# fanzhongyi/diffusion

Hardware: AMD Instinct MI355X
Metric: U-Net training images/sec @256 (SD-2-base U-Net, precomputed latents 4x32x32) (higher is better)
Workload: dtype bf16; 1 GPU; SD-2-base U-Net train step, latents 4x32x32, text 77x1024, batch 256/GPU (global 256), microbatch 256, AdamW, dp1; global_batch=256, microbatch=256, parallelism=dp1, params=865910724

## Files before the change

### diffusion_amd/_lib.py

```python
from __future__ import annotations

import ctypes as C
import os

_HERE = os.path.dirname(os.path.abspath(__file__))
LIB_PATH = os.path.join(_HERE, os.environ.get('DA_LIB_ALT') or 'libdiffusion_amd.so')

_vp, _l, _i, _f, _fp, _ll = C.c_void_p, C.c_long, C.c_int, C.c_float, C.c_void_p, C.c_void_p



class DaWgradItem(C.Structure):
    _fields_ = [('dY', C.c_void_p), ('lddy', C.c_long), ('X', C.c_void_p), ('ldx', C.c_long), ('dW', C.c_void_p),
                ('dbias', C.c_void_p), ('N', C.c_int), ('Cin', C.c_int)]


SIGNATURES = {
    'da_gemm_nt': [_vp, _l, _vp, _vp, _l, _fp, _vp, _l, _vp, _l, _i, _i, _i, _i, _i, _i, _i, _i, _i, _i, _i, _f, _fp, _l,
                   _vp],
    'da_set_option': [C.c_char_p, _i],
    'da_gemm_nt_variant_for': [_i, _i, _i, _i, _l],
    'da_gemm_nt_geglu': [_vp, _l, _vp, _vp, _l, _vp, _l, _fp, _i, _i, _i, _vp],
    'da_gemm_nt_geglu_bwd': [_vp, _l, _vp, _vp, _l, _vp, _l, _i, _i, _i, _vp],
    'da_gemm_tn_wgrad': [_vp, _l, _vp, _l, _fp, _fp, _fp, _i, _i, _i, _i, _i, _i, _i, _i, _i, _fp, _l, _vp],
    'da_gemm_tn_variant_for': [_i, _i, _i, _i, _i, _i, _i, _i, _i],
    'da_gemm_tn_wgrad_group': [C.POINTER(DaWgradItem), _i, _i, _fp, _l, _vp],
    'da_gemm_tn_group_plan': [C.POINTER(DaWgradItem), _i, _i, _l, C.POINTER(_i), _i, C.POINTER(_i)],
    'da_attn_fwd': [_vp, _l, _vp, _l, _vp, _l, _vp, _l, _fp, _i, _i, _i, _i, _f, _vp],
    'da_attn_fwd_causal': [_vp, _l, _vp, _l, _vp, _l, _vp, _l, _fp, _i, _i, _i, _f, _vp],
    'da_attn_fwd_wide': [_vp, _l, _vp, _l, _vp, _l, _vp, _l, _fp, _i, _i, _i, _i, _i, _f, _vp],
    'da_attn_bwd': [_vp, _l, _vp, _l, _vp, _l, _vp, _l, _vp, _l, _fp, _fp, _vp, _l, _vp, _l, _vp, _l, _i, _i, _i, _i,
                    _f, _vp],
    'da_norm_scratch_floats': [_i, _i, _i],
    'da_groupnorm_fwd': [_vp, _l, _vp, _l, _fp, _fp, _fp, _fp, _fp, _i, _i, _i, _i, _f, _i, _vp],
    'da_groupnorm_bwd': [_vp, _l, _vp, _l, _vp, _l, _vp, _l, _fp, _fp, _fp, _fp, _fp, _fp, _fp, _i, _i, _i, _i, _i,
                         _vp],
# ... 85 lines not shown
```

### diffusion_amd/csrc/gemm_nt.hip

```cpp
#include <string.h>

#include "common.hpp"
#include "diffusion_amd.h"

namespace {

struct GemmNTParams {
  const bf16* A;
  const bf16* W;
  void* C;
  const float* bias;
  const bf16* rowbias;
  const bf16* R;
  long lda, ldc, ldrb, ldr;
  int M, N, K, Cin;
  int Hin, Win, Hout, Wout;
  int ksize, mode;
  int out_fp32;
  float alpha;
  int tiles_m, tiles_n;
};

constexpr int BM = 128, BN = 128, BK = 64;
constexpr int STAGE_BYTES = (BM + BN) * BK * 2;
// ... 193 lines not shown
      }
    }
  }
}

}

int da_gemm_nt_v2_dispatch(int variant, int splits, float* ws, const void* A, long lda, const void* W, void* C, long ldc, const float* bias,
                           const void* rowbias, long ldrb, const void* R, long ldr, int M, int N, int K, int Cin,
                           int Hin, int Win, int Hout, int Wout, int ksize, int mode, int out_fp32, float alpha,
                           hipStream_t stream);

int da_gemm_nt_v3_try(const void* A, long lda, const void* W, void* C, long ldc, const float* bias, const void* R, long ldr,
                      int M, int N, int K, hipStream_t stream);
extern int g_nt_stream, g_nt_stream_lw;
int da_gemm_nt_ws_try(const void* A, long lda, const void* W, const float* bias, const void* R, long ldr, void* C, long ldc,
                      int M, int N, int K, hipStream_t stream);
extern int g_nt_ws;

extern int g_tn_variant;
extern int g_nt_korder;
extern int g_nt_persist;
extern int g_reserve_cus;
extern int g_nt_persist_conv;
extern int g_nt_de;
extern int g_grad_overwrite;
extern int g_attn_fused_bwd;
extern int g_tn_ring, g_tn_ungroup;
extern int g_gn_resident, g_gn_resident_form, g_gn_resident_min_slab;
int da_usable_cus(int cus);
// ... 52 lines not shown
        best_v = f.variant;
        best_s = s;
      }
    }
  }
  *splits = best_s;
  if (best_v == 12 && (g_nt_mfma32 == 1 || (g_nt_mfma32 < 0 && K <= 320))) return 15;
  return best_v;
}

extern "C" int da_gemm_nt_variant_for(int M, int N, int K, int Cin, long ws_floats) {
  int s;
  return pick_nt_variant(M, N, K, Cin, ws_floats, &s);
}

extern "C" int da_set_option(const char* key, int value) {
  if (key && !strcmp(key, "gemm_nt_variant")) {
    g_nt_variant = value;
    return DA_OK;
  }
  if (key && !strcmp(key, "gemm_nt_splitk")) {
    g_nt_splitk = value;
    return DA_OK;
  }
  if (key && !strcmp(key, "gemm_nt_dispatch")) {
    g_nt_dispatch = value;
    return DA_OK;
  }
  if (key && !strcmp(key, "gemm_nt_persist")) {
    g_nt_persist = value;
// ... 28 lines not shown
    if (value != 0 && value != 1) return DA_ERR_SHAPE;
    g_tn_ungroup = value;
    return DA_OK;
  }
  if (key && !strcmp(key, "gemm_nt_stream_lw")) {
    if (value != 4 && value != 16) return DA_ERR_SHAPE;
    g_nt_stream_lw = value;
    return DA_OK;
  }
  if (key && !strcmp(key, "gemm_nt_stream")) {
    g_nt_stream = value;
    return DA_OK;
  }
  if (key && !strcmp(key, "gemm_nt_de")) {
    g_nt_de = value;
    return DA_OK;
  }
  if (key && !strcmp(key, "gemm_nt_persist_conv")) {
    g_nt_persist_conv = value;
    return DA_OK;
  }
  if (key && !strcmp(key, "gn_resident")) {
    if (value < 0) return DA_ERR_SHAPE;
    g_gn_resident = value;
    return DA_OK;
  }
  if (key && !strcmp(key, "gn_resident_min_slab")) {
    if (value < 0) return DA_ERR_SHAPE;
    g_gn_resident_min_slab = value;
    return DA_OK;
// ... 29 lines not shown
  if (Hout <= 0 || Wout <= 0 || (M % (Hout * Wout))) return DA_ERR_SHAPE;
  if (R && (ldr & 7)) return DA_ERR_SHAPE;
  if (rowbias && (ldrb & 7)) return DA_ERR_SHAPE;
  if (g_nt_ws && g_nt_variant == 0 && ksize == 1 && mode == 0 && !out_fp32 && alpha == 1.0f && !rowbias) {
    const int rc = da_gemm_nt_ws_try(A, lda, W, bias, R, ldr, C, ldc, M, N, K, stream);
    if (rc >= 0) return rc;
  }
  if (g_nt_stream && g_nt_variant == 0 && ksize == 1 && mode == 0 && !out_fp32 && alpha == 1.0f && !rowbias &&
      (g_nt_stream == 2 || (K <= 640 && (long)((M + 127) / 128) * ((N + 319) / 320) >= 512))) {
    const int rc = da_gemm_nt_v3_try(A, lda, W, C, ldc, bias, R, ldr, M, N, K, stream);
    if (rc >= 0) return rc;
  }
  {
    int splits = 1;
    const int variant = pick_nt_variant(M, N, K, Cin, splitk_ws ? splitk_ws_floats : 0, &splits);
    if (variant != 1)
      return da_gemm_nt_v2_dispatch(variant, splits, splitk_ws, A, lda, W, C, ldc, bias, rowbias, ldrb, R, ldr, M, N, K, Cin, Hin, Win,
                                    Hout, Wout, ksize, mode, out_fp32, alpha, stream);
  }
  GemmNTParams p;
  p.A = (const bf16*)A; p.W = (const bf16*)W; p.C = C; p.bias = bias;
  p.rowbias = (const bf16*)rowbias; p.R = (const bf16*)R;
  p.lda = lda; p.ldc = ldc; p.ldrb = ldrb; p.ldr = ldr;
  p.M = M; p.N = N; p.K = K; p.Cin = Cin;
  p.Hin = Hin; p.Win = Win; p.Hout = Hout; p.Wout = Wout;
  p.ksize = ksize; p.mode = mode; p.out_fp32 = out_fp32; p.alpha = alpha;
  p.tiles_m = (M + BM - 1) / BM;
  p.tiles_n = (N + BN - 1) / BN;
  static unsigned long long attr_done = 0;
  if (da_ensure_dyn_smem((const void*)gemm_nt_kernel, SMEM_BYTES, &attr_done) != DA_OK) return DA_ERR_LAUNCH;
  hipLaunchKernelGGL(gemm_nt_kernel, dim3(p.tiles_m * p.tiles_n), dim3(256), SMEM_BYTES, stream, p);
  DA_CHECK_LAUNCH();
  return DA_OK;
}
```

### diffusion_amd/csrc/gemm_nt_v2.hip

```cpp
#include "common.hpp"
#include "diffusion_amd.h"
#ifndef NT2_NT
#define NT2_NT 0
#endif
#if NT2_NT
#define NTST st8_nt
#else
#define NTST st8
#endif


#ifndef NT2_CT
#define NT2_CT 1
#endif

int g_nt_persist = -1;
int g_reserve_cus = 0;
int g_nt_persist_conv = 1;
int g_nt_de = 1;
int da_usable_cus(int cus) {
  int n = cus - g_reserve_cus;
  return n < 32 ? 32 : n;
}

namespace {

struct GemmNT2Params {
  const bf16* A;
  const bf16* W;
  void* C;
  const float* bias;
  const bf16* rowbias;
  const bf16* R;
  long lda, ldc, ldrb, ldr;
  int M, N, K, Cin;
  int Hin, Win, Hout, Wout;
  int ksize, mode;
  int out_fp32;
  float alpha;
  int tiles_m, tiles_n;
  int splits, ksteps_per_split;
  long slab_stride;
  bf16* G;
  long ldg;
  int inner;
  int total_blocks;
  FastDiv div_hw, div_w;
  FastDiv div_nblk, div_tn;
  int korder;
};

__device__ __attribute__((aligned(256))) unsigned char g_zero_page[256];

template <int BK>
DEVINL int swz_key(int row) { return BK == 64 ? ((row >> 1) & 7) : ((row >> 2) & 3); }
template <int BK>
DEVINL int swz2(int row, int chunk) { return row * (BK * 2) + ((chunk ^ swz_key<BK>(row)) << 4); }

DEVINL void lds_barrier() {
  asm volatile("s_waitcnt lgkmcnt(0)" ::: "memory");
  __builtin_amdgcn_s_barrier();
  asm volatile("" ::: "memory");
}

// ... 4 lines not shown
    if (threadIdx.x == 0 && g_stamp_buf) g_stamp_buf[(long)vblock * 16 + (i)] = __builtin_amdgcn_s_memtime(); \
  } while (0)
extern "C" int da_debug_set_stamps(void* buf) {
  return hipMemcpyToSymbol(HIP_SYMBOL(g_stamp_buf), &buf, sizeof(buf)) == hipSuccess ? 0 : -1;
}
#else
#define STAMP(i) do {} while (0)
#endif

DEVINL void glds16(const void* gsrc, char* lds_dst) {
  __builtin_amdgcn_global_load_lds((const __attribute__((address_space(1))) void*)gsrc,
                                   (__attribute__((address_space(3))) void*)lds_dst, 16, 0, 0);
}

template <int MT, int NT, int WM, int WN, int BK, bool UPS, int GEGLU, bool EARLY, int MF = 16, bool PERSIST = EARLY, bool DE = false,
          bool HASR = false>
DEVINL void nt2_tile(const GemmNT2Params& p, const int vblock0, char* smem) {
  constexpr int NW = WM * WN;
  constexpr bool CT = MF == 16 && GEGLU == 0 && ((NT2_CT && !EARLY) || DE);
  static_assert(!DE || (MF == 16 && GEGLU == 0 && ((NT % 2) == 0 || (MT % 2) == 0)), "direct epilogue: 16x16 tiles in pairs");
  constexpr int V2_BM = MF * MT * WM, V2_BK = BK;
  static_assert((NW == 16 || NW == 8 || NW == 4) && (BK == 64 || BK == 32), "wave grid");
  static_assert(MF == 16 || (MF == 32 && GEGLU == 0 && BK == 64), "MFMA shape");
  constexpr int BN = MF * NT * WN;
  constexpr int SR = MF == 16 ? 16 : 8;
  constexpr int RG = 512 / BK;
  constexpr int LR = BK / 8;
  constexpr int AJ = V2_BM / RG / NW;
  constexpr int BGROUPS = BN / RG;
  constexpr int BJ = (BGROUPS + NW - 1) / NW;
  constexpr int A_BYTES = V2_BM * V2_BK * 2;
  constexpr int B_BYTES = BN * V2_BK * 2;
// ... 10 lines not shown
  const int wm = wave / WN, wn = wave % WN;
  auto task_of = [&](int ln, int pss, int tasks) {
    const bool ragged_last = (tasks % (64 * WN)) != 0 && pss == (tasks + 64 * WN - 1) / (64 * WN) - 1;
    const int slot = ragged_last ? (wn + WN - (wm * WN / 4) % WN) % WN : wn;
    return slot * 64 + ln + 64 * WN * pss;
  };
  auto fresh_lane = [&]() {
    int ln = lane;
    asm volatile("" : "+v"(ln));
    return ln;
  };
  STAMP(0);

  const int nblk = p.tiles_m * p.tiles_n;
  int split, tn, m0, n0;
  auto locate = [&](int vb) {
    split = (PERSIST && !EARLY) ? (int)fdiv((unsigned)vb, p.div_nblk) : vb / nblk;
    int bid = vb - split * nblk;
    const int q = nblk >> 3, r = nblk & 7;
    const int xcd = bid & 7, idx = bid >> 3;
    bid = (xcd < r ? xcd * (q + 1) : r * (q + 1) + (xcd - r) * q) + idx;
    const int tm = (PERSIST && !EARLY) ? (int)fdiv((unsigned)bid, p.div_tn) : bid / p.tiles_n;
    tn = bid - tm * p.tiles_n;
    m0 = tm * V2_BM;
    n0 = tn * BN;
  };
  auto wrow = [&](int c) {
    if constexpr (GEGLU == 1) return c < BN / 2 ? tn * (BN / 2) + c : p.inner + tn * (BN / 2) + (c - BN / 2);
    else return n0 + c;
  };
  const int HWo = p.Hout * p.Wout;
// ... 25 lines not shown
#pragma unroll
  for (int j = 0; j < AJ; ++j) {
    const int row = (wave * AJ + j) * RG + lrow;
    const int m = m0 + row;
    const bool mval = m < p.M;
    if constexpr (EARLY) {
#ifdef NT2_EXP_AHOT
      aoff[j] = (unsigned)(row) * (unsigned)(p.lda * 2) + (lchunk ^ swz_key<BK>(row)) * 16;
#else
      aoff[j] = (unsigned)(mval ? m : 0) * (unsigned)(p.lda * 2) + (lchunk ^ swz_key<BK>(row)) * 16;
#endif
      continue;
    }
    const int mm = mval ? m : 0;
    int b, rem, oh;
    if constexpr (PERSIST) {
      b = (int)fdiv((unsigned)mm, p.div_hw);
      rem = mm - b * HWo;
      oh = (int)fdiv((unsigned)rem, p.div_w);
    } else {
      b = mm / HWo;
      rem = mm - b * HWo;
      oh = rem / p.Wout;
    }
    const int ow = rem - oh * p.Wout;
    unsigned mask = ((oh & 1) << 16) | ((ow & 1) << 17);
    for (int t = 0; t < ntaps; ++t) {
      const int r = (PCONV || p.ksize == 3) ? t / 3 : 0, s2 = (PCONV || p.ksize == 3) ? t - 3 * r : 0;
      const int th = oh * gmul + r - pad, tw = ow * gmul + s2 - pad;
      const bool ok = mval && (unsigned)th < (unsigned)hlim && (unsigned)tw < (unsigned)wlim && !((th | tw) & pmask);
      mask |= (ok ? 1u : 0u) << t;
    }
    const int bh = (oh * gmul - pad) >> gshift, bw = (ow * gmul - pad) >> gshift;
    if constexpr (PERSIST && !UPS) {
// ... 1 lines not shown
      if (j == 0) amask[0] = mask & 0x1ffu;
      else amask[0] |= (mask & 0x1ffu) << (9 * j);
      continue;
    }
    amask[j] = mask;
    abase[j] = p.A + ((long)(b * p.Hin * p.Win) + (long)bh * p.Win + bw) * p.lda + (lchunk ^ swz_key<BK>(row)) * 8;
  }
#pragma unroll
  for (int j = 0; j < BJ; ++j) {
    const int g = wave + NW * j;
    const int row = g * RG + lrow;
    const int n = min(wrow(row), p.N - 1);
    woff[j] = ((unsigned)n * (unsigned)p.K + (lchunk ^ swz_key<BK>(row)) * 8) * 2;
  }

  const int kstep_begin = split * p.ksteps_per_split;
  nk = min(p.ksteps_per_split, nk_total - kstep_begin);
  if (tap_inner) {
    const int ch = kstep_begin / ntaps;
    tap = kstep_begin - ch * ntaps;
    c0 = ch * V2_BK;
  } else {
    const int kb = kstep_begin * V2_BK;
    tap = kb / p.Cin;
    c0 = kb - tap * p.Cin;
  }
  };
  auto issue = [&](int stage, bool live) {
    char* Ab = smem + stage * STAGE;
    char* Bb = Ab + A_BYTES;
// ... 30 lines not shown
        const long soff = (long)(dr * p.Win + ds) * p.lda + c0;
        const void* src = (amask[j] & tapbit) ? (const void*)(abase[j] + soff) : (const void*)zero;
        glds16(src, Ab + (wave * AJ + j) * 1024);
      }
    }
    const char* wb = reinterpret_cast<const char*>(p.W + (live ? tap * p.Cin + c0 : 0));
#pragma unroll
    for (int j = 0; j < BJ; ++j) {
      const int g = wave + NW * j;
      if constexpr (PERSIST && !EARLY) {
        if (BGROUPS % NW == 0 || g < BGROUPS) glds16(wb + (size_t)j * (NW * RG) * p.K * 2 + woff[0], Bb + g * 1024);
      } else {
        if (BGROUPS % NW == 0 || g < BGROUPS) glds16(wb + woff[j], Bb + g * 1024);
      }
    }
    const int tap_n = tap + 1, c_n = c0 + V2_BK;
    const bool wrap_t = tap_n >= ntaps, wrap_c = c_n >= p.Cin;
    if (tap_inner) {
      tap = wrap_t ? 0 : tap_n;
      c0 = wrap_t ? c_n : c0;
    } else {
      c0 = wrap_c ? 0 : c_n;
      tap = wrap_c ? tap_n : tap;
    }
  };

  typedef float accv_t __attribute__((ext_vector_type(MF == 16 ? 4 : 16)));
  accv_t acc[MT][NT];

  auto compute_half = [&](int stage, int s) {
    const char* Ab = smem + stage * STAGE;
    const char* Bb = Ab + A_BYTES;
// ... 96 lines not shown

  auto epilogue = [&](const int m0e, const int n0e, const int tne, const int splite, const int bbuf) {
  if constexpr (DE) {
    typedef unsigned u32x2_t __attribute__((ext_vector_type(2)));
    constexpr int NPJ = NT / 2;
    constexpr bool ODD = (NT & 1) != 0;
    constexpr int IH = ODD ? ((MT / 2 + 1) / 2) * 2 : (MT + 1) / 2;
    const int ln = fresh_lane();
    char* const cb = reinterpret_cast<char*>(p.C);
    const char* const rb = reinterpret_cast<const char*>(p.R);
    const int lrow = wm * (16 * MT) + (ln & 15), lq = (ln >> 4) & 1, lcol = wn * (16 * NT) + 8 * (ln >> 5);
    auto row_of = [&](int i) { return m0e + lrow + i * 16; };
    auto col_of = [&](int pj) { return n0e + lcol + 32 * pj + 16 * lq; };
    auto row5_of = [&](int i) { return m0e + lrow + (i - 1 + lq) * 16; };
    const int col5 = n0e + lcol + 16 * (NT - 1);
    u32x4 rin[MT][NPJ > 0 ? NPJ : 1], rin5[MT];
    auto fetch = [&](const int i_lo, const int i_hi) {
#pragma unroll
      for (int i = 0; i < MT; ++i) {
        if (i < i_lo || i >= i_hi) continue;
        const unsigned mo = (unsigned)min(row_of(i), p.M - 1) * (unsigned)(p.ldr * 2);
#pragma unroll
        for (int pj = 0; pj < NPJ; ++pj)
          rin[i][pj] = *reinterpret_cast<const u32x4*>(rb + (mo + (unsigned)min(col_of(pj), p.N - 8) * 2u));
        if constexpr (ODD) {
          if (i & 1)
            rin5[i] = *reinterpret_cast<const u32x4*>(rb + ((unsigned)min(row5_of(i), p.M - 1) * (unsigned)(p.ldr * 2) +
                                                            (unsigned)min(col5, p.N - 8) * 2u));
        }
      }
    };
    auto finish = [&](accv_t a, accv_t b, const u32x4 r, const int ma, const int mb, const int na, const int nb) {
      if (p.rowbias) {
        const int ia = (PERSIST && !EARLY) ? (int)fdiv((unsigned)min(ma, p.M - 1), p.div_hw) : min(ma, p.M - 1) / HWo;
        const int ib = (PERSIST && !EARLY) ? (int)fdiv((unsigned)min(mb, p.M - 1), p.div_hw) : min(mb, p.M - 1) / HWo;
        const bf16x4 ra = *reinterpret_cast<const bf16x4*>(p.rowbias + (long)ia * p.ldrb + min(na, p.N - 4));
        const bf16x4 rb4 = *reinterpret_cast<const bf16x4*>(p.rowbias + (long)ib * p.ldrb + min(nb, p.N - 4));
#pragma unroll
        for (int e = 0; e < 4; ++e) {
          a[e] += bf2f(ra[e]);
          b[e] += bf2f(rb4[e]);
        }
      }
      if constexpr (HASR) {
        const u32x2_t s0 = __builtin_amdgcn_permlane16_swap(r[0], r[2], false, false);
        const u32x2_t s1 = __builtin_amdgcn_permlane16_swap(r[1], r[3], false, false);
        a[0] += __builtin_bit_cast(float, s0[0] << 16);
// ... 17 lines not shown
#pragma unroll
    for (int i = 0; i < MT; ++i) {
      if constexpr (HASR) {
        if (i == IH) fetch(IH, MT);
      }
      const int m = row_of(i);
      const int ma = m0e + wm * (16 * MT) + i * 16 + (ln & 15);
#pragma unroll
      for (int pj = 0; pj < NPJ; ++pj) {
        const int n = col_of(pj);
        const int na = n0e + wn * (16 * NT) + 32 * pj + aq;
        const u32x4 o = finish(acc[i][2 * pj], acc[i][2 * pj + 1], rin[i][pj], ma, ma, na, na + 16);
#ifdef NT2_EXP_NOSTORE
        asm volatile("" ::"v"(o));
#else
        if (m < p.M && n < p.N) *reinterpret_cast<u32x4*>(cb + ((unsigned)m * (unsigned)(p.ldc * 2) + (unsigned)n * 2u)) = o;
#endif
      }
      if constexpr (ODD) {
        if (i & 1) {
          const int m5 = row5_of(i);
          const int na = n0e + wn * (16 * NT) + 16 * (NT - 1) + aq;
          const u32x4 o = finish(acc[i - 1][NT - 1], acc[i][NT - 1], rin5[i], ma - 16, ma, na, na);
#ifdef NT2_EXP_NOSTORE
          asm volatile("" ::"v"(o));
#else
          if (m5 < p.M && col5 < p.N) *reinterpret_cast<u32x4*>(cb + ((unsigned)m5 * (unsigned)(p.ldc * 2) + (unsigned)col5 * 2u)) = o;
#endif
        }
      }
    }
    STAMP(4);
    return;
  }
  const float* bias_lds = reinterpret_cast<const float*>(smem + BIAS_OFF + bbuf * (BN * 4));
  float* const strips = reinterpret_cast<float*>(smem + STRIP_OFF);
  const int el = fresh_lane();
  if constexpr (GEGLU == 1) {
    static_assert(BN == 320 && !UPS, "GEGLU tile = 160 value + 160 gate columns");
    constexpr int GLD = BN + 4, GSTRIP = 16 * GLD, HC = BN / 2;
    constexpr int GTASKS = 16 * (HC / 8), GPASSES = (GTASKS + 64 * WN - 1) / (64 * WN);
    const int mrow0g = m0e + wm * (16 * MT);
// ... 227 lines not shown
        locate(vnext);
        load_bias(bbuf ^ 1);
        describe();
        issue(0, true);
      }
      STAMP(8);
      epilogue(m0e, n0e, tne, splite, bbuf);
      STAMP(12);
      if (!more) break;
      vblock = vnext;
    }
  }
}

template <int MT, int NT, int WM, int WN, int BK, bool UPS, int GEGLU = 0, bool EARLY = false, int MF = 16, bool PERSIST = EARLY, bool DE = false,
          bool HASR = false>
__global__ __launch_bounds__(64 * WM * WN, (WM * WN == 16 ? 4 : 2)) void gemm_nt2_kernel(GemmNT2Params p) {
  extern __shared__ __attribute__((aligned(16))) char smem[];
  nt2_tile<MT, NT, WM, WN, BK, UPS, GEGLU, EARLY, MF, PERSIST, DE, HASR>(p, blockIdx.x, smem);
}

__global__ void splitk_finalize_kernel(GemmNT2Params p, const float* ws) {
  const int nvec = p.N >> 3;
  const long total = (long)p.M * nvec;
  const int HWo = p.Hout * p.Wout;
  for (long i = (long)blockIdx.x * blockDim.x + threadIdx.x; i < total; i += (long)gridDim.x * blockDim.x) {
    const long m = i / nvec;
    const int n = (int)(i - m * nvec) * 8;
    float v[8] = {0.f, 0.f, 0.f, 0.f, 0.f, 0.f, 0.f, 0.f};
#pragma unroll 4
    for (int s = 0; s < p.splits; ++s) {
      const float* src = ws + s * p.slab_stride + m * p.N + n;
      const f32x4 a = *reinterpret_cast<const f32x4*>(src), b = *reinterpret_cast<const f32x4*>(src + 4);
#pragma unroll
// ... 89 lines not shown
        hipLaunchKernelGGL((gemm_nt2_kernel<MT, NT, WM, WN, BK, UPS, 0, EARLY, MF, PERSIST, true, true>), dim3(grid), dim3(NTHREADS), SMEM, stream, p);
      } else {
        if (da_ensure_dyn_smem((const void*)gemm_nt2_kernel<MT, NT, WM, WN, BK, UPS, 0, EARLY, MF, PERSIST, true, false>, SMEM, &attr_done_de[0]) != DA_OK)
          return DA_ERR_LAUNCH;
        hipLaunchKernelGGL((gemm_nt2_kernel<MT, NT, WM, WN, BK, UPS, 0, EARLY, MF, PERSIST, true, false>), dim3(grid), dim3(NTHREADS), SMEM, stream, p);
      }
      DA_CHECK_LAUNCH();
      return DA_OK;
    }
  }
  hipLaunchKernelGGL((gemm_nt2_kernel<MT, NT, WM, WN, BK, UPS, 0, EARLY, MF, PERSIST>), dim3(grid), dim3(NTHREADS), SMEM, stream, p);
  DA_CHECK_LAUNCH();
  return DA_OK;
}

template <int GM>
int launch_v2_geglu(GemmNT2Params p, hipStream_t stream) {
  constexpr int BN = 320, STAGE = 256 * 64 * 2 + BN * 64 * 2, STRIPS = 4 * 16 * (BN + 4) * 4;
  constexpr int SMEM = (STAGE + STRIPS > 2 * STAGE ? STAGE + STRIPS : 2 * STAGE) + 2 * BN * 4;
  static_assert(SMEM <= 160 * 1024, "LDS");
  p.tiles_m = (p.M + 255) / 256;
  p.tiles_n = GM == 1 ? (p.inner + BN / 2 - 1) / (BN / 2) : (p.inner + BN - 1) / BN;
  p.splits = 1;
  p.ksteps_per_split = p.K / 64;
  static unsigned long long attr_done = 0;
  if (da_ensure_dyn_smem((const void*)gemm_nt2_kernel<4, 5, 4, 4, 64, false, GM, true>, SMEM, &attr_done) != DA_OK) return DA_ERR_LAUNCH;
  p.total_blocks = p.tiles_m * p.tiles_n;
  p.div_nblk = make_fastdiv((unsigned)p.total_blocks);
  p.div_tn = make_fastdiv((unsigned)p.tiles_n);
  if (p.total_blocks >= (1 << 20) || p.M >= (1 << 24)) return DA_ERR_SHAPE;
// ... 30 lines not shown
  GemmNT2Params p;
  p.A = (const bf16*)A; p.W = (const bf16*)W; p.C = C; p.bias = bias;
  p.rowbias = (const bf16*)rowbias; p.R = (const bf16*)R;
  p.lda = lda; p.ldc = ldc; p.ldrb = ldrb; p.ldr = ldr;
  p.M = M; p.N = N; p.K = K; p.Cin = Cin;
  p.Hin = Hin; p.Win = Win; p.Hout = Hout; p.Wout = Wout;
  p.ksize = ksize; p.mode = mode; p.out_fp32 = out_fp32; p.alpha = alpha;
  p.tiles_m = p.tiles_n = 0;
  p.splits = 1; p.ksteps_per_split = 0; p.slab_stride = 0;
  p.G = nullptr; p.ldg = 0; p.inner = 0;
  p.korder = g_nt_korder;
  p.total_blocks = 0;
  p.div_hw = make_fastdiv((unsigned)(Hout * Wout));
  p.div_w = make_fastdiv((unsigned)Wout);
  p.div_nblk = p.div_tn = make_fastdiv(1u);
  if (variant == 10) return launch_v2<8, 5, 2, 4, 64>(p, splits, ws, stream);
  if (variant == 11) return launch_v2<4, 10, 2, 2, 32>(p, 1, ws, stream);
  if (variant == 12) return launch_v2<4, 5, 4, 4, 64>(p, splits, ws, stream);
  if (variant == 15) return launch_v2<1, 5, 8, 2, 64, 32>(p, splits, ws, stream);
  if (variant == 16) return launch_v2<2, 5, 4, 2, 64, 32>(p, splits, ws, stream);
  if (variant == 18) return launch_v2<3, 4, 8, 2, 64>(p, splits, ws, stream);
  if (variant == 14) return launch_v2<4, 4, 4, 4, 64>(p, splits, ws, stream);
  return variant == 5 ? launch_v2<4, 5, 4, 2, 64>(p, splits, ws, stream) : launch_v2<4, 4, 4, 2, 64>(p, splits, ws, stream);
}

int da_gemm_nt_geglu_ws_try(const void* A, long lda, const void* W, const float* bias, void* F, long ldf, void* G, long ldg,
                            int M, int inner, int K, hipStream_t stream);

extern "C" int da_gemm_nt_geglu(const void* A, long lda, const void* W, void* F, long ldf, void* G, long ldg,
                                const float* bias, int M, int inner, int K, hipStream_t stream) {
  DA_CLEAR_ERR();
  if (M <= 0 || inner <= 0 || K <= 0) return DA_ERR_SHAPE;
  if ((inner % 160) || (K % 64) || (lda & 7) || (ldf & 7) || (ldg & 7)) return DA_ERR_SHAPE;
  if ((long)M * lda * 2 >= (1L << 32) || (long)inner * K * 4 >= (1L << 32)) return DA_ERR_SHAPE;
  {
    const int rc = da_gemm_nt_geglu_ws_try(A, lda, W, bias, F, ldf, G, ldg, M, inner, K, stream);
    if (rc >= 0) return rc;
  }
  GemmNT2Params p;
  p.A = (const bf16*)A; p.W = (const bf16*)W; p.C = F; p.bias = bias;
  p.rowbias = nullptr; p.R = nullptr;
  p.lda = lda; p.ldc = ldf; p.ldrb = 0; p.ldr = 0;
  p.M = M; p.N = 2 * inner; p.K = K; p.Cin = K;
  p.Hin = 1; p.Win = 1; p.Hout = 1; p.Wout = 1;
  p.ksize = 1; p.mode = 0; p.out_fp32 = 0; p.alpha = 1.0f;
  p.tiles_m = p.tiles_n = 0;
  p.splits = 1; p.ksteps_per_split = 0; p.slab_stride = 0;
  p.G = (bf16*)G; p.ldg = ldg; p.inner = inner; p.korder = 0; p.total_blocks = 0;
  p.div_hw = p.div_w = p.div_nblk = p.div_tn = make_fastdiv(1u);
  return launch_v2_geglu<1>(p, stream);
}

extern "C" int da_gemm_nt_geglu_bwd(const void* dY, long lddy, const void* Wt, const void* F, long ldf, void* dF, long lddf,
                                    int M, int inner, int K, hipStream_t stream) {
  DA_CLEAR_ERR();
  if (M <= 0 || inner <= 0 || K <= 0) return DA_ERR_SHAPE;
  if ((inner % 320) || (K % 64) || (lddy & 7) || (ldf & 7) || (lddf & 7)) return DA_ERR_SHAPE;
  if ((long)M * lddy * 2 >= (1L << 32) || (long)inner * K * 2 >= (1L << 32)) return DA_ERR_SHAPE;
  GemmNT2Params p;
  p.A = (const bf16*)dY; p.W = (const bf16*)Wt; p.C = dF; p.bias = nullptr;
  p.rowbias = nullptr; p.R = nullptr;
  p.lda = lddy; p.ldc = lddf; p.ldrb = 0; p.ldr = 0;
  p.M = M; p.N = inner; p.K = K; p.Cin = K;
  p.Hin = 1; p.Win = 1; p.Hout = 1; p.Wout = 1;
  p.ksize = 1; p.mode = 0; p.out_fp32 = 0; p.alpha = 1.0f;
  p.tiles_m = p.tiles_n = 0;
  p.splits = 1; p.ksteps_per_split = 0; p.slab_stride = 0;
  p.G = (bf16*)const_cast<void*>(F); p.ldg = ldf; p.inner = inner; p.korder = 0; p.total_blocks = 0;
  p.div_hw = p.div_w = p.div_nblk = p.div_tn = make_fastdiv(1u);
  return launch_v2_geglu<2>(p, stream);
}
```

### diffusion_amd/models/unet.py

```python
from __future__ import annotations

import math
import os
from dataclasses import dataclass
from typing import Dict, List, Optional, Tuple

import torch
import torch.nn as nn

from .. import ops
from ..ops import BF16, F32, Geom


@dataclass
class UNetConfig:
    in_channels: int = 4
    out_channels: int = 4
    block_out_channels: Tuple[int, ...] = (320, 640, 1280, 1280)
    attention_head_dim: Tuple[int, ...] = (5, 10, 20, 20)
    cross_attention_dim: int = 1024
    layers_per_block: int = 2
    norm_num_groups: int = 32
    norm_eps: float = 1e-5
    sample_size: int = 64
# ... 838 lines not shown
                self._wgrad(dpred, a, m.gw, g3, dbias=self.V('conv_out.bias').g, scratch=self._scratch)
                da = self._bf(B * H * W, m.C)
                ops.gemm_nt(dpred, m.wt, da, g3)
                dh = self._gn_bwd(h, da, None, 'conv_norm_out', st, B, H * W, 1)
            elif kind == 'resnet':
                dh = self._resnet_bwd(sv, dh)
                lo = off(sv[0] + '.norm1.weight')
            elif kind == 'transformer':
                dh = self._transformer_bwd(sv, dh)
                lo = off(sv[0] + '.norm.weight')
            elif kind == 'up':
                key, x, B, rh, rw = sv
                lo = off(key + '.weight')
                m = self.M(key + '.weight')
                self._wgrad(dh, x, m.gw, Geom.up(B, rh, rw), dbias=self.V(key + '.bias').g, scratch=self._scratch)
                dup = self._bf(B * 4 * rh * rw, m.C)
                ops.gemm_nt(dh, m.wt, dup, Geom.conv(B, 2 * rh, 2 * rw))
                dx = self._bf(B * rh * rw, m.C)
                ops.upsample2x_bwd(dup, dx, B, rh, rw, m.C)
                dh = dx
            elif kind == 'cat':
                s, cb = sv
                dskip[s] = dh[:, cb:]
                dh = dh[:, :cb]
            elif kind == 'skip':
                (s,) = sv
                tot = self._bf(*dh.shape)
                ops.add(dh, dskip.pop(s), tot)
                dh = tot
            elif kind == 'down':
                key, x, B, rh, rw = sv
                lo = off(key + '.weight')
                m = self.M(key + '.weight')
                self._wgrad(dh, x, m.gw, Geom.down(B, rh, rw), dbias=self.V(key + '.bias').g, scratch=self._scratch)
# ... 63 lines not shown
```

### diffusion_amd/ops.py

```python
from __future__ import annotations

import ctypes
import os
from typing import Optional, Tuple

import torch

from . import _lib

BF16 = torch.bfloat16
F32 = torch.float32


def _stream() -> int:
    return torch.cuda.current_stream().cuda_stream


SPLITK_WS = None


PROFILE = None


class _Timed:
# ... 122 lines not shown
                14: 'gemm_nt2_kernel<4,4,4,4>', 15: 'gemm_nt2_kernel<1,5,8,2,mf32>', 16: 'gemm_nt2_kernel<2,5,4,2,mf32>',
                18: 'gemm_nt2_kernel<3,4,8,2>'}[v]
        ws = _opt('gemm_nt_ws', 1)
        ws_bn = 320 if (K == 320 and (ws & 1) and N <= 1280) else 128 if (K == 640 and (ws & 2) and N <= 1024) else 0
        if (ws_bn and _opt('gemm_nt_variant', 0) == 0 and N % ws_bn == 0 and M % 32 == 0 and (M // 32) * (N // ws_bn) >= 8 * 256
                and g.ksize == 1 and g.mode == 0 and not out_fp32 and alpha == 1.0 and rowbias is None):
            name = 'gemm_nt_ws_kernel'
    with _Timed(name, flops, (M, N, K, g.ksize, g.mode)):
        _lib.call('da_gemm_nt', a_ptr, lda, w_ptr, c_ptr, ldc, _vec(bias, N, 'bias'), rb_ptr, ldrb, r_ptr, ldr, M, N,
                  K, Cin, g.Hin, g.Win, g.Hout, g.Wout, g.ksize, g.mode, int(out_fp32), float(alpha),
                  SPLITK_WS.data_ptr() if SPLITK_WS is not None else 0,
                  SPLITK_WS.numel() if SPLITK_WS is not None else 0, _stream())
    return out


def geglu_fusable(inner: int, K: int) -> bool:
    return inner % 160 == 0 and K % 64 == 0


def gemm_nt_geglu(A, W, F, G, bias):
    a_ptr, lda = _mat(A, BF16, 'A')
    w_ptr, ldw = _mat(W, BF16, 'W')
    f_ptr, ldf = _mat(F, BF16, 'F')
    g_ptr, ldg = _mat(G, BF16, 'G')
    M, K = A.shape
    inner = G.shape[1]
    if tuple(W.shape) != (2 * inner, K) or ldw != K or tuple(F.shape) != (M, 2 * inner) or G.shape[0] != M:
        raise ValueError('gemm_nt_geglu: shape mismatch')
    if not geglu_fusable(inner, K):
        raise ValueError(f'gemm_nt_geglu needs inner % 160 == 0 and K % 64 == 0, got {inner}, {K}')
# ... 660 lines not shown
```

### include/diffusion_amd.h

```cpp
#ifndef DIFFUSION_AMD_H
#define DIFFUSION_AMD_H

#ifdef __cplusplus
extern "C" {
#endif

typedef struct ihipStream_t* da_stream_t;

int da_gemm_nt(const void* A, long lda, const void* W, void* C, long ldc, const float* bias, const void* rowbias,
               long ldrb, const void* R, long ldr, int M, int N, int K, int Cin, int Hin, int Win, int Hout, int Wout,
               int ksize, int mode, int out_fp32, float alpha, float* splitk_ws, long splitk_ws_floats,
               da_stream_t stream);

int da_gemm_nt_geglu(const void* A, long lda, const void* W, void* F, long ldf, void* G, long ldg, const float* bias,
                     int M, int inner, int K, da_stream_t stream);

int da_gemm_nt_geglu_bwd(const void* dY, long lddy, const void* Wt, const void* F, long ldf, void* dF, long lddf, int M,
                         int inner, int K, da_stream_t stream);

int da_set_option(const char* key, int value);
int da_gemm_nt_variant_for(int M, int N, int K, int Cin, long splitk_ws_floats);

int da_gemm_tn_wgrad(const void* dY, long lddy, const void* X, long ldx, float* dW, float* dbias, float* scratch, int M,
                     int N, int Cin, int Hin, int Win, int Hout, int Wout, int ksize, int mode, float* split_ws,
                     long split_ws_floats, da_stream_t stream);

int da_gemm_tn_variant_for(int M, int N, int Cin, int Hin, int Win, int Hout, int Wout, int ksize, int mode);

typedef struct DaWgradItem {
  const void* dY;
  long lddy;
  const void* X;
  long ldx;
  float* dW;
  float* dbias;
  int N;
// ... 145 lines not shown
```

Baseline: 1517 images/sec.

## Add parity-class upsample conv and fold upsample backward into dgrad GEMM

Measured after the change: 1523 images/sec, median of 6. No clear change (+0.4%).

```diff
diff --git a/diffusion_amd/_lib.py b/diffusion_amd/_lib.py
--- a/diffusion_amd/_lib.py
+++ b/diffusion_amd/_lib.py
@@ -20,6 +20,8 @@
                    _vp],
     'da_set_option': [C.c_char_p, _i],
     'da_gemm_nt_variant_for': [_i, _i, _i, _i, _l],
+    'da_gemm_nt_form_launches': [_i],
+    'da_gemm_nt_up_fold': [_vp, _l, _vp, _vp, _l, _fp, _i, _i, _i, _i, _i, _l, _vp],
     'da_gemm_nt_geglu': [_vp, _l, _vp, _vp, _l, _vp, _l, _fp, _i, _i, _i, _vp],
     'da_gemm_nt_geglu_bwd': [_vp, _l, _vp, _vp, _l, _vp, _l, _i, _i, _i, _vp],
     'da_gemm_tn_wgrad': [_vp, _l, _vp, _l, _fp, _fp, _fp, _i, _i, _i, _i, _i, _i, _i, _i, _i, _fp, _l, _vp],
diff --git a/diffusion_amd/csrc/gemm_nt.hip b/diffusion_amd/csrc/gemm_nt.hip
--- a/diffusion_amd/csrc/gemm_nt.hip
+++ b/diffusion_amd/csrc/gemm_nt.hip
@@ -231,6 +231,13 @@
 int da_gemm_nt_v3_try(const void* A, long lda, const void* W, void* C, long ldc, const float* bias, const void* R, long ldr,
                       int M, int N, int K, hipStream_t stream);
 extern int g_nt_stream, g_nt_stream_lw;
+int da_gemm_nt_s2c_try(const void* A, long lda, const void* W, void* C, long ldc, const float* bias, const void* rowbias, const void* R,
+                       int M, int N, int K, int Cin, int Hin, int Win, int Hout, int Wout, int ksize, int mode, int out_fp32, float alpha,
+                       hipStream_t stream);
+int da_gemm_nt_upf_try(const void* dY, long lddy, const void* Wt, void* dX, long lddx, const float* bias, int B, int H, int W, int N, int Cin,
+                       hipStream_t stream);
+extern int g_nt_s2_classes, g_nt_up_fold;
+extern long g_nt_s2_launches, g_nt_upf_launches;
 int da_gemm_nt_ws_try(const void* A, long lda, const void* W, const float* bias, const void* R, long ldr, void* C, long ldc,
                       int M, int N, int K, hipStream_t stream);
 extern int g_nt_ws;
@@ -313,6 +320,11 @@
   return pick_nt_variant(M, N, K, Cin, ws_floats, &s);
 }
 
+extern "C" int da_gemm_nt_form_launches(int form) {
+  if (form != 0 && form != 1) return -1;
+  return (int)((form ? g_nt_upf_launches : g_nt_s2_launches) & 0x7fffffff);
+}
+
 extern "C" int da_set_option(const char* key, int value) {
   if (key && !strcmp(key, "gemm_nt_variant")) {
     g_nt_variant = value;
@@ -371,6 +383,16 @@
   }
   if (key && !strcmp(key, "gemm_nt_de")) {
     g_nt_de = value;
+    return DA_OK;
+  }
+  if (key && !strcmp(key, "gemm_nt_s2_classes")) {
+    if (value != 0 && value != 1) return DA_ERR_SHAPE;
+    g_nt_s2_classes = value;
+    return DA_OK;
+  }
+  if (key && !strcmp(key, "gemm_nt_up_fold")) {
+    if (value != 0 && value != 1) return DA_ERR_SHAPE;
+    g_nt_up_fold = value;
     return DA_OK;
   }
   if (key && !strcmp(key, "gemm_nt_persist_conv")) {
@@ -430,6 +452,11 @@
   {
     int splits = 1;
     const int variant = pick_nt_variant(M, N, K, Cin, splitk_ws ? splitk_ws_floats : 0, &splits);
+    if (g_nt_s2_classes && g_nt_variant == 0 && mode == 2 && splits == 1 &&
+        (variant == 4 || variant == 5 || variant == 12 || variant == 14 || variant == 18)) {
+      const int rc = da_gemm_nt_s2c_try(A, lda, W, C, ldc, bias, rowbias, R, M, N, K, Cin, Hin, Win, Hout, Wout, ksize, mode, out_fp32, alpha, stream);
+      if (rc >= 0) return rc;
+    }
     if (variant != 1)
       return da_gemm_nt_v2_dispatch(variant, splits, splitk_ws, A, lda, W, C, ldc, bias, rowbias, ldrb, R, ldr, M, N, K, Cin, Hin, Win,
                                     Hout, Wout, ksize, mode, out_fp32, alpha, stream);
@@ -449,3 +476,15 @@
   DA_CHECK_LAUNCH();
   return DA_OK;
 }
+
+extern "C" int da_gemm_nt_up_fold(const void* dY, long lddy, const void* Wt, void* dX, long lddx, const float* bias, int B, int H, int W, int N,
+                                  int Cin, long splitk_ws_floats, hipStream_t stream) {
+  DA_CLEAR_ERR();
+  if (B <= 0 || H <= 0 || W <= 0 || N <= 0 || Cin <= 0 || (long)B * 4 * H * W >= (1L << 31)) return DA_ERR_SHAPE;
+  if ((N & 7) || (Cin & 7) || (lddy & 7) || (lddx & 7)) return DA_ERR_SHAPE;
+  if (!g_nt_up_fold || g_nt_variant != 0) return -1;
+  int splits = 1;
+  const int variant = pick_nt_variant(B * 4 * H * W, N, 9 * Cin, Cin, splitk_ws_floats, &splits);
+  if (splits != 1 || !(variant == 4 || variant == 5 || variant == 12 || variant == 14 || variant == 18)) return -1;
+  return da_gemm_nt_upf_try(dY, lddy, Wt, dX, lddx, bias, B, H, W, N, Cin, stream);
+}
diff --git a/diffusion_amd/csrc/gemm_nt_v2.hip b/diffusion_amd/csrc/gemm_nt_v2.hip
--- a/diffusion_amd/csrc/gemm_nt_v2.hip
+++ b/diffusion_amd/csrc/gemm_nt_v2.hip
@@ -18,6 +18,9 @@
 int g_reserve_cus = 0;
 int g_nt_persist_conv = 1;
 int g_nt_de = 1;
+int g_nt_s2_classes = 1;
+int g_nt_up_fold = 1;
+long g_nt_s2_launches = 0, g_nt_upf_launches = 0;
 int da_usable_cus(int cus) {
   int n = cus - g_reserve_cus;
   return n < 32 ? 32 : n;
@@ -48,6 +51,7 @@
   FastDiv div_hw, div_w;
   FastDiv div_nblk, div_tn;
   int korder;
+  int s2_tmc;
 };
 
 __device__ __attribute__((aligned(256))) unsigned char g_zero_page[256];
@@ -82,8 +86,10 @@
 }
 
 template <int MT, int NT, int WM, int WN, int BK, bool UPS, int GEGLU, bool EARLY, int MF = 16, bool PERSIST = EARLY, bool DE = false,
-          bool HASR = false>
+          bool HASR = false, bool S2C = false, bool UPF = false>
 DEVINL void nt2_tile(const GemmNT2Params& p, const int vblock0, char* smem) {
+  static_assert(!S2C || (DE && !HASR && !PERSIST && !EARLY && !UPS && GEGLU == 0 && BK == 64), "parity-class form");
+  static_assert(!UPF || (DE && !HASR && !S2C && !EARLY && !UPS && GEGLU == 0 && BK == 64), "block-sum form");
   constexpr int NW = WM * WN;
   constexpr bool CT = MF == 16 && GEGLU == 0 && ((NT2_CT && !EARLY) || DE);
   static_assert(!DE || (MF == 16 && GEGLU == 0 && ((NT % 2) == 0 || (MT % 2) == 0)), "direct epilogue: 16x16 tiles in pairs");
@@ -124,7 +130,22 @@
 
   const int nblk = p.tiles_m * p.tiles_n;
   int split, tn, m0, n0;
+  int cls = 0;
   auto locate = [&](int vb) {
+    if constexpr (S2C) {
+      const int nct = p.s2_tmc * p.tiles_n;
+      cls = vb / nct;
+      int bid = vb - cls * nct;
+      const int q = nct >> 3, r = nct & 7;
+      const int xcd = bid & 7, idx = bid >> 3;
+      bid = (xcd < r ? xcd * (q + 1) : r * (q + 1) + (xcd - r) * q) + idx;
+      const int tm = bid / p.tiles_n;
+      split = 0;
+      tn = bid - tm * p.tiles_n;
+      m0 = tm * V2_BM;
+      n0 = tn * BN;
+      return;
+    }
     split = (PERSIST && !EARLY) ? (int)fdiv((unsigned)vb, p.div_nblk) : vb / nblk;
     int bid = vb - split * nblk;
     const int q = nblk >> 3, r = nblk & 7;
@@ -180,10 +201,28 @@
     }
     const int mm = mval ? m : 0;
     int b, rem, oh;
-    if constexpr (PERSIST) {
+    if constexpr (UPF) {
+      const int ql = mm >> 2, hwl = HWo >> 2, wl = p.Wout >> 1;
+      int lh;
+      if constexpr (PERSIST) {
+        b = (int)fdiv((unsigned)ql, p.div_hw);
+        lh = (int)fdiv((unsigned)(ql - b * hwl), p.div_w);
+      } else {
+        b = ql / hwl;
+        lh = (ql - b * hwl) / wl;
+      }
+      oh = 2 * lh + ((mm >> 1) & 1);
+      rem = oh * p.Wout + 2 * (ql - b * hwl - lh * wl) + (mm & 1);
+    } else if constexpr (PERSIST) {
       b = (int)fdiv((unsigned)mm, p.div_hw);
       rem = mm - b * HWo;
       oh = (int)fdiv((unsigned)rem, p.div_w);
+    } else if constexpr (S2C) {
+      const int hwl = p.Hin * p.Win;
+      b = mm / hwl;
+      const int reml = mm - b * hwl, lh = reml / p.Win;
+      oh = 2 * lh + (~cls & 1);
+      rem = oh * p.Wout + 2 * (reml - lh * p.Win) + ((~cls >> 1) & 1);
     } else {
       b = mm / HWo;
       rem = mm - b * HWo;
@@ -215,6 +254,13 @@
     woff[j] = ((unsigned)n * (unsigned)p.K + (lchunk ^ swz_key<BK>(row)) * 8) * 2;
   }
 
+  if constexpr (S2C) {
+    const int py = ~cls & 1, px = (~cls >> 1) & 1;
+    nk = (1 + py) * (1 + px) * (p.Cin / V2_BK);
+    tap = (py ? 0 : 3) + (px ? 0 : 1);
+    c0 = 0;
+    return;
+  }
   const int kstep_begin = split * p.ksteps_per_split;
   nk = min(p.ksteps_per_split, nk_total - kstep_begin);
   if (tap_inner) {
@@ -275,8 +321,26 @@
         if (BGROUPS % NW == 0 || g < BGROUPS) glds16(wb + woff[j], Bb + g * 1024);
       }
     }
-    const int tap_n = tap + 1, c_n = c0 + V2_BK;
-    const bool wrap_t = tap_n >= ntaps, wrap_c = c_n >= p.Cin;
+    const int c_n = c0 + V2_BK;
+    const bool wrap_c = c_n >= p.Cin;
+    if constexpr (S2C) {
+      const int py = ~cls & 1, px = (~cls >> 1) & 1;
+      int tap_n = (py ? 0 : 3) + (px ? 0 : 1);
+      bool wrap_t = false;
+      if (px && s2 == 0) tap_n = tap + 2;
+      else if (py && r == 0) tap_n = 6 + (px ? 0 : 1);
+      else wrap_t = true;
+      if (tap_inner) {
+        tap = tap_n;
+        c0 = wrap_t ? c_n : c0;
+      } else {
+        c0 = wrap_c ? 0 : c_n;
+        tap = wrap_c ? tap_n : tap;
+      }
+      return;
+    }
+    const int tap_n = tap + 1;
+    const bool wrap_t = tap_n >= ntaps;
     if (tap_inner) {
       tap = wrap_t ? 0 : tap_n;
       c0 = wrap_t ? c_n : c0;
@@ -403,6 +467,16 @@
     auto col_of = [&](int pj) { return n0e + lcol + 32 * pj + 16 * lq; };
     auto row5_of = [&](int i) { return m0e + lrow + (i - 1 + lq) * 16; };
     const int col5 = n0e + lcol + 16 * (NT - 1);
+    auto crow = [&](int m) {
+      if constexpr (S2C) {
+        const int g = m / p.Win;
+        return (unsigned)((2 * g + (~cls & 1)) * p.Wout + 2 * (m - g * p.Win) + ((~cls >> 1) & 1));
+      } else if constexpr (UPF) {
+        return (unsigned)(m >> 2);
+      } else {
+        return (unsigned)m;
+      }
+    };
     u32x4 rin[MT][NPJ > 0 ? NPJ : 1], rin5[MT];
     auto fetch = [&](const int i_lo, const int i_hi) {
 #pragma unroll
@@ -419,7 +493,23 @@
         }
       }
     };
+    auto block_sum = [&](const float v) {
+      const int x = __builtin_bit_cast(int, bf2f(f2bf(v)));
+      float sum = 0.f;
+      sum += __builtin_bit_cast(float, __builtin_amdgcn_update_dpp(0, x, 0x00, 0xf, 0xf, false));
+      sum += __builtin_bit_cast(float, __builtin_amdgcn_update_dpp(0, x, 0x55, 0xf, 0xf, false));
+      sum += __builtin_bit_cast(float, __builtin_amdgcn_update_dpp(0, x, 0xaa, 0xf, 0xf, false));
+      sum += __builtin_bit_cast(float, __builtin_amdgcn_update_dpp(0, x, 0xff, 0xf, 0xf, false));
+      return sum;
+    };
     auto finish = [&](accv_t a, accv_t b, const u32x4 r, const int ma, const int mb, const int na, const int nb) {
+      if constexpr (UPF) {
+#pragma unroll
+        for (int e = 0; e < 4; ++e) {
+          a[e] = block_sum(a[e]);
+          b[e] = block_sum(b[e]);
+        }
+      }
       if (p.rowbias) {
         const int ia = (PERSIST && !EARLY) ? (int)fdiv((unsigned)min(ma, p.M - 1), p.div_hw) : min(ma, p.M - 1) / HWo;
         const int ib = (PERSIST && !EARLY) ? (int)fdiv((unsigned)min(mb, p.M - 1), p.div_hw) : min(mb, p.M - 1) / HWo;
@@ -467,7 +557,7 @@
 #ifdef NT2_EXP_NOSTORE
         asm volatile("" ::"v"(o));
 #else
-        if (m < p.M && n < p.N) *reinterpret_cast<u32x4*>(cb + ((unsigned)m * (unsigned)(p.ldc * 2) + (unsigned)n * 2u)) = o;
+        if (m < p.M && n < p.N && (!UPF || (ln & 3) == 0)) *reinterpret_cast<u32x4*>(cb + (crow(m) * (unsigned)(p.ldc * 2) + (unsigned)n * 2u)) = o;
 #endif
       }
       if constexpr (ODD) {
@@ -478,7 +568,7 @@
 #ifdef NT2_EXP_NOSTORE
           asm volatile("" ::"v"(o));
 #else
-          if (m5 < p.M && col5 < p.N) *reinterpret_cast<u32x4*>(cb + ((unsigned)m5 * (unsigned)(p.ldc * 2) + (unsigned)col5 * 2u)) = o;
+          if (m5 < p.M && col5 < p.N && (!UPF || (ln & 3) == 0)) *reinterpret_cast<u32x4*>(cb + (crow(m5) * (unsigned)(p.ldc * 2) + (unsigned)col5 * 2u)) = o;
 #endif
         }
       }
@@ -736,10 +826,10 @@
 }
 
 template <int MT, int NT, int WM, int WN, int BK, bool UPS, int GEGLU = 0, bool EARLY = false, int MF = 16, bool PERSIST = EARLY, bool DE = false,
-          bool HASR = false>
+          bool HASR = false, bool S2C = false, bool UPF = false>
 __global__ __launch_bounds__(64 * WM * WN, (WM * WN == 16 ? 4 : 2)) void gemm_nt2_kernel(GemmNT2Params p) {
   extern __shared__ __attribute__((aligned(16))) char smem[];
-  nt2_tile<MT, NT, WM, WN, BK, UPS, GEGLU, EARLY, MF, PERSIST, DE, HASR>(p, blockIdx.x, smem);
+  nt2_tile<MT, NT, WM, WN, BK, UPS, GEGLU, EARLY, MF, PERSIST, DE, HASR, S2C, UPF>(p, blockIdx.x, smem);
 }
 
 __global__ void splitk_finalize_kernel(GemmNT2Params p, const float* ws) {
@@ -859,6 +949,65 @@
   return DA_OK;
 }
 
+int launch_v2_s2c(GemmNT2Params p, hipStream_t stream) {
+  constexpr int BM = 256, BN = 320, STAGE = BM * 64 * 2 + BN * 64 * 2, SMEM = 2 * STAGE + BN * 4;
+  if (p.mode != 2 || p.ksize != 3 || p.R || p.rowbias || p.out_fp32 || p.alpha != 1.0f) return -1;
+  if (p.Hout != 2 * p.Hin || p.Wout != 2 * p.Win || (p.M % (p.Hout * p.Wout)) || (p.Cin % 64) || p.K != 9 * p.Cin) return -1;
+  if ((p.N % 8) || (p.ldc % 8) || ((uintptr_t)p.C & 15) || (long)p.M * p.ldc * 2 >= (1L << 32) || (long)p.N * p.K * 2 >= (1L << 32)) return -1;
+  p.M /= 4;
+  p.s2_tmc = (p.M + BM - 1) / BM;
+  p.tiles_m = 4 * p.s2_tmc;
+  p.tiles_n = (p.N + BN - 1) / BN;
+  p.splits = 1;
+  p.ksteps_per_split = p.K / 64;
+  p.slab_stride = 0;
+  p.total_blocks = p.tiles_m * p.tiles_n;
+  static unsigned long long attr_done = 0;
+  if (da_ensure_dyn_smem((const void*)gemm_nt2_kernel<4, 5, 4, 4, 64, false, 0, false, 16, false, true, false, true>, SMEM, &attr_done) != DA_OK)
+    return DA_ERR_LAUNCH;
+  hipLaunchKernelGGL((gemm_nt2_kernel<4, 5, 4, 4, 64, false, 0, false, 16, false, true, false, true>), dim3(p.total_blocks), dim3(1024), SMEM, stream, p);
+  DA_CHECK_LAUNCH();
+  ++g_nt_s2_launches;
+  return DA_OK;
+}
+
+template <bool PERS>
+int launch_v2_upf_form(GemmNT2Params p, hipStream_t stream) {
+  constexpr int BM = 256, BN = 320, STAGE = BM * 64 * 2 + BN * 64 * 2, STRIPS = 4 * 16 * (BN + 4) * 4;
+  constexpr int SMEM = PERS ? (STAGE + STRIPS > 2 * STAGE ? STAGE + STRIPS : 2 * STAGE) + 2 * BN * 4 : 2 * STAGE + BN * 4;
+  static_assert(SMEM <= 160 * 1024, "LDS");
+  p.tiles_m = (p.M + BM - 1) / BM;
+  p.tiles_n = (p.N + BN - 1) / BN;
+  p.splits = 1;
+  p.ksteps_per_split = p.K / 64;
+  p.slab_stride = 0;
+  p.total_blocks = p.tiles_m * p.tiles_n;
+  p.div_nblk = make_fastdiv((unsigned)p.total_blocks);
+  p.div_tn = make_fastdiv((unsigned)p.tiles_n);
+  p.div_hw = make_fastdiv((unsigned)(p.Hout * p.Wout / 4));
+  p.div_w = make_fastdiv((unsigned)(p.Wout / 2));
+  if (PERS && p.total_blocks >= (1 << 20)) return -1;
+  static unsigned long long attr_done = 0;
+  if (da_ensure_dyn_smem((const void*)gemm_nt2_kernel<4, 5, 4, 4, 64, false, 0, false, 16, PERS, true, false, false, true>, SMEM, &attr_done) != DA_OK)
+    return DA_ERR_LAUNCH;
+  const int grid = PERS ? persistent_grid(p.total_blocks) : p.total_blocks;
+  hipLaunchKernelGGL((gemm_nt2_kernel<4, 5, 4, 4, 64, false, 0, false, 16, PERS, true, false, false, true>), dim3(grid), dim3(1024), SMEM, stream, p);
+  DA_CHECK_LAUNCH();
+  ++g_nt_upf_launches;
+  return DA_OK;
+}
+
+int launch_v2_upf(const GemmNT2Params& p, hipStream_t stream) {
+  if (p.mode != 0 || p.ksize != 3 || p.R || p.rowbias || p.out_fp32 || p.alpha != 1.0f) return -1;
+  if (p.Hin != p.Hout || p.Win != p.Wout || (p.Hout & 1) || (p.Wout & 1) || (p.M % (p.Hout * p.Wout)) || (p.Cin % 64) || p.K != 9 * p.Cin) return -1;
+  if ((p.N % 8) || (p.ldc % 8) || ((uintptr_t)p.C & 15) || (long)(p.M / 4) * p.ldc * 2 >= (1L << 32) || (long)p.N * p.K * 2 >= (1L << 32)) return -1;
+  const long tiles = (long)((p.M + 255) / 256) * ((p.N + 319) / 320);
+  if (g_nt_persist_conv && g_nt_persist != 0 && tiles > da_usable_cus(256) && p.N % 320 == 0 && p.M < (1 << 24) &&
+      (long)p.M * p.Hout * p.Wout < (1L << 40) && (long)(p.M / (p.Hout * p.Wout)) * p.Hin * p.Win * p.lda * 2 < (1L << 32))
+    return launch_v2_upf_form<true>(p, stream);
+  return launch_v2_upf_form<false>(p, stream);
+}
+
 template <int GM>
 int launch_v2_geglu(GemmNT2Params p, hipStream_t stream) {
   constexpr int BN = 320, STAGE = 256 * 64 * 2 + BN * 64 * 2, STRIPS = 4 * 16 * (BN + 4) * 4;
@@ -919,6 +1068,9 @@
   p.div_hw = make_fastdiv((unsigned)(Hout * Wout));
   p.div_w = make_fastdiv((unsigned)Wout);
   p.div_nblk = p.div_tn = make_fastdiv(1u);
+  p.s2_tmc = 0;
+  if (variant == -2) return launch_v2_s2c(p, stream);
+  if (variant == -3) return launch_v2_upf(p, stream);
   if (variant == 10) return launch_v2<8, 5, 2, 4, 64>(p, splits, ws, stream);
   if (variant == 11) return launch_v2<4, 10, 2, 2, 32>(p, 1, ws, stream);
   if (variant == 12) return launch_v2<4, 5, 4, 4, 64>(p, splits, ws, stream);
@@ -927,6 +1079,19 @@
   if (variant == 18) return launch_v2<3, 4, 8, 2, 64>(p, splits, ws, stream);
   if (variant == 14) return launch_v2<4, 4, 4, 4, 64>(p, splits, ws, stream);
   return variant == 5 ? launch_v2<4, 5, 4, 2, 64>(p, splits, ws, stream) : launch_v2<4, 4, 4, 2, 64>(p, splits, ws, stream);
+}
+
+int da_gemm_nt_s2c_try(const void* A, long lda, const void* W, void* C, long ldc, const float* bias, const void* rowbias, const void* R,
+                       int M, int N, int K, int Cin, int Hin, int Win, int Hout, int Wout, int ksize, int mode, int out_fp32, float alpha,
+                       hipStream_t stream) {
+  return da_gemm_nt_v2_dispatch(-2, 1, nullptr, A, lda, W, C, ldc, bias, rowbias, 0, R, 0, M, N, K, Cin, Hin, Win, Hout, Wout, ksize, mode,
+                                out_fp32, alpha, stream);
+}
+
+int da_gemm_nt_upf_try(const void* dY, long lddy, const void* Wt, void* dX, long lddx, const float* bias, int B, int H, int W, int N, int Cin,
+                       hipStream_t stream) {
+  return da_gemm_nt_v2_dispatch(-3, 1, nullptr, dY, lddy, Wt, dX, lddx, bias, nullptr, 0, nullptr, 0, B * 4 * H * W, N, 9 * Cin, Cin, 2 * H, 2 * W,
+                                2 * H, 2 * W, 3, 0, 0, 1.0f, stream);
 }
 
 int da_gemm_nt_geglu_ws_try(const void* A, long lda, const void* W, const float* bias, void* F, long ldf, void* G, long ldg,
@@ -951,7 +1116,7 @@
   p.ksize = 1; p.mode = 0; p.out_fp32 = 0; p.alpha = 1.0f;
   p.tiles_m = p.tiles_n = 0;
   p.splits = 1; p.ksteps_per_split = 0; p.slab_stride = 0;
-  p.G = (bf16*)G; p.ldg = ldg; p.inner = inner; p.korder = 0; p.total_blocks = 0;
+  p.G = (bf16*)G; p.ldg = ldg; p.inner = inner; p.korder = 0; p.total_blocks = 0; p.s2_tmc = 0;
   p.div_hw = p.div_w = p.div_nblk = p.div_tn = make_fastdiv(1u);
   return launch_v2_geglu<1>(p, stream);
 }
@@ -971,7 +1136,7 @@
   p.ksize = 1; p.mode = 0; p.out_fp32 = 0; p.alpha = 1.0f;
   p.tiles_m = p.tiles_n = 0;
   p.splits = 1; p.ksteps_per_split = 0; p.slab_stride = 0;
-  p.G = (bf16*)const_cast<void*>(F); p.ldg = ldf; p.inner = inner; p.korder = 0; p.total_blocks = 0;
+  p.G = (bf16*)const_cast<void*>(F); p.ldg = ldf; p.inner = inner; p.korder = 0; p.total_blocks = 0; p.s2_tmc = 0;
   p.div_hw = p.div_w = p.div_nblk = p.div_tn = make_fastdiv(1u);
   return launch_v2_geglu<2>(p, stream);
 }
diff --git a/diffusion_amd/models/unet.py b/diffusion_amd/models/unet.py
--- a/diffusion_amd/models/unet.py
+++ b/diffusion_amd/models/unet.py
@@ -876,10 +876,11 @@
                 lo = off(key + '.weight')
                 m = self.M(key + '.weight')
                 self._wgrad(dh, x, m.gw, Geom.up(B, rh, rw), dbias=self.V(key + '.bias').g, scratch=self._scratch)
-                dup = self._bf(B * 4 * rh * rw, m.C)
-                ops.gemm_nt(dh, m.wt, dup, Geom.conv(B, 2 * rh, 2 * rw))
                 dx = self._bf(B * rh * rw, m.C)
-                ops.upsample2x_bwd(dup, dx, B, rh, rw, m.C)
+                if not ops.gemm_nt_up_fold(dh, m.wt, dx, B, rh, rw):
+                    dup = self._bf(B * 4 * rh * rw, m.C)
+                    ops.gemm_nt(dh, m.wt, dup, Geom.conv(B, 2 * rh, 2 * rw))
+                    ops.upsample2x_bwd(dup, dx, B, rh, rw, m.C)
                 dh = dx
             elif kind == 'cat':
                 s, cb = sv
diff --git a/diffusion_amd/ops.py b/diffusion_amd/ops.py
--- a/diffusion_amd/ops.py
+++ b/diffusion_amd/ops.py
@@ -160,6 +160,27 @@
     return out
 
 
+def gemm_nt_up_fold(dY, Wt, dx, B, H, W):
+    dy_ptr, lddy = _mat(dY, BF16, 'dY')
+    w_ptr, ldw = _mat(Wt, BF16, 'Wt')
+    dx_ptr, lddx = _mat(dx, BF16, 'dx')
+    N, K = Wt.shape
+    Cin = dY.shape[1]
+    M = B * 4 * H * W
+    if ldw != K or K != 9 * Cin or dY.shape[0] != M or tuple(dx.shape) != (B * H * W, N):
+        raise ValueError('gemm_nt_up_fold: shape mismatch')
+    tm = _Timed('gemm_nt2_kernel<4,5,4,4>', 2.0 * M * N * K, (M, N, K, 3, 'up_fold'))
+    tm.__enter__()
+    rc = _lib.load().da_gemm_nt_up_fold(dy_ptr, lddy, w_ptr, dx_ptr, lddx, 0, B, H, W, N, Cin,
+                                        SPLITK_WS.numel() if SPLITK_WS is not None else 0, _stream())
+    if rc == -1:
+        return False
+    tm.__exit__()
+    if rc != 0:
+        raise RuntimeError(f'da_gemm_nt_up_fold failed: {rc}')
+    return True
+
+
 def geglu_fusable(inner: int, K: int) -> bool:
     return inner % 160 == 0 and K % 64 == 0
 
diff --git a/include/diffusion_amd.h b/include/diffusion_amd.h
--- a/include/diffusion_amd.h
+++ b/include/diffusion_amd.h
@@ -20,6 +20,9 @@
 
 int da_set_option(const char* key, int value);
 int da_gemm_nt_variant_for(int M, int N, int K, int Cin, long splitk_ws_floats);
+int da_gemm_nt_form_launches(int form);
+int da_gemm_nt_up_fold(const void* dY, long lddy, const void* Wt, void* dX, long lddx, const float* bias, int B, int H, int W, int N,
+                       int Cin, long splitk_ws_floats, da_stream_t stream);
 
 int da_gemm_tn_wgrad(const void* dY, long lddy, const void* X, long ldx, float* dW, float* dbias, float* scratch, int M,
                      int N, int Cin, int Hin, int Win, int Hout, int Wout, int ksize, int mode, float* split_ws,
```
